# Samaretas/global-motion-estimation

Hardware: AMD Instinct MI355X
Metric: frame-pairs/s + achieved HBM GB/s, 720x480 bs=16 sw=16 exhaustive (higher is better)
Workload: dtype u8; 1 GPU; 720x480 synthetic luma, bs=16 sw=16 exhaustive MAE (BASELINE configs[1]); frame_distance=1, streams_per_gpu=1, collective=none, exchange=none in this run, multi_gpu_measured_by_builder=False

## Files before the change

global-motion-estimation_amd/csrc/bbme_sea.hip:

```cpp
#include "bbme_sea_common.h"

namespace {

using namespace sea;

constexpr int GUARD_NONE = 0, GUARD_ROWS = 1, GUARD_ALL = 2;
constexpr uint32_t PENALTY = 1u << 17;
constexpr uint32_t FIRST_INVALID_KEY = 65536u << 13;
template <int R, int GUARD>
__device__ __forceinline__ void lower_bounds(const uint64_t* sp0, int XQ, int prow, int q, uint32_t a01, uint32_t a23,
                                             int lo_r, int hi_r, int lo_c, int hi_c, uint32_t (&pkey)[R])
{
    constexpr bool SKIP = GUARD == GUARD_ALL && R >= 4;
#pragma unroll
    for (int k = 0; k < R; ++k) pkey[k] = 0xFFFFFFFFu;
    constexpr uint32_t penalty = PENALTY;
    uint32_t seed[R];
#pragma unroll
    for (int i = 0; i < R; ++i) {
        const int ri = prow * R + i;
        seed[i] = (GUARD == GUARD_NONE || SKIP || (ri >= lo_r && ri <= hi_r)) ? 0u : penalty;
    }
    const int nlo = lo_c - q * 4 * R, nhi = hi_c - q * 4 * R;
    const uint64_t* top = sp0;
    const uint64_t* bot = sp0 + 8 * XQ;
#pragma unroll
    for (int i = 0; i < R; ++i) {
        const int ri = prow * R + i;
        if (!SKIP || (ri >= lo_r && ri <= hi_r)) {
            uint64_t t[R + 2], b[R + 2];
#pragma unroll
            for (int k = 0; k < R + 2; ++k) { t[k] = top[k]; b[k] = bot[k]; }
#pragma unroll
            for (int k = 0; k < R; ++k) {
                if (SKIP && (4 * k > nhi || 4 * k + 3 < nlo)) continue;
#pragma unroll
                for (int e = 0; e < 4; ++e) {
                    if (SKIP && (4 * k + e < nlo || 4 * k + e > nhi)) continue;
                    const uint32_t sel = (e & 1) ? 0x07060302u : 0x05040100u;
                    const uint32_t tp = __builtin_amdgcn_perm((uint32_t)(t[k + 2] >> (32 * (e >> 1))), (uint32_t)(t[k] >> (32 * (e >> 1))), sel);
                    const uint32_t bt = __builtin_amdgcn_perm((uint32_t)(b[k + 2] >> (32 * (e >> 1))), (uint32_t)(b[k] >> (32 * (e >> 1))), sel);
                    const uint32_t start = (GUARD != GUARD_ALL || SKIP || 4 * k + e <= nhi) ? seed[i] : penalty;
                    const uint32_t lb = __builtin_amdgcn_sad_u16(tp, a01, __builtin_amdgcn_sad_u16(bt, a23, start));
                    pkey[k] = min(pkey[k], (lb << 13) + (uint32_t)((4 * k + e) * R + i));
                }
            }
        }
        top += XQ;
        bot += XQ;
    }
    if constexpr (GUARD != GUARD_NONE && !SKIP) {
#pragma unroll
        for (int k = 0; k < R; ++k)
            if (pkey[k] >= FIRST_INVALID_KEY || (GUARD == GUARD_ALL && 4 * k < nlo)) pkey[k] = 0xFFFFFFFFu;
    }
}

template <int R>
__device__ __forceinline__ uint32_t eval_patch_quad(const SeaGeo& d, int H, int W, const uint32_t* win, const uint32_t* anchor, uint32_t ent,
                                                    bool active, int sub, int trow, int bcol0, int NC)
{
    const int w2 = ent >> 25, l2 = (ent >> 19) & 63, k2 = (ent >> 16) & 7;
    const int wr2 = div_small(w2, d.magic_tc), wc2 = w2 - wr2 * d.tc;
    const int prow2 = l2 >> 2, q2 = l2 & 3;
    uint64_t acc[R];
#pragma unroll
    for (int i = 0; i < R; ++i) acc[i] = 0;
    if (active) {
        const uint32_t* lrow = win + (16 * wr2 + prow2 * R + 4 * sub) * d.pitch_dw + wc2 * 4 + q2 * R + k2;
        const uint32_t* an = anchor + w2 * ANCHOR_STRIDE + 16 * sub;
#pragma unroll
        for (int t = 0; t < R + 3; ++t) {
            uint64_t w[4];
#pragma unroll
            for (int s = 0; s < 4; ++s) w[s] = *(const u64_a4*)(lrow + t * d.pitch_dw + s);
#pragma unroll
            for (int i = 0; i < R; ++i) {
                const int a = t - i;
                if (a < 0 || a > 3) continue;
                const u32x4 ar = *(const u32x4*)(an + a * 4);
#pragma unroll
                for (int j = 0; j < 4; ++j)
                    acc[i] = __builtin_amdgcn_qsad_pk_u16_u8(w[j], ar[j], acc[i]);
            }
        }
    }
#pragma unroll
    for (int i = 0; i < R; ++i) {
        uint32_t lo = (uint32_t)acc[i], hi = (uint32_t)(acc[i] >> 32);
        lo += (uint32_t)__builtin_amdgcn_update_dpp(0, (int)lo, 0xB1, 0xF, 0xF, false);
        hi += (uint32_t)__builtin_amdgcn_update_dpp(0, (int)hi, 0xB1, 0xF, 0xF, false);
        lo += (uint32_t)__builtin_amdgcn_update_dpp(0, (int)lo, 0x4E, 0xF, 0xF, false);
        hi += (uint32_t)__builtin_amdgcn_update_dpp(0, (int)hi, 0x4E, 0xF, 0xF, false);
        asm volatile("" : "+v"(lo), "+v"(hi));
        acc[i] = ((uint64_t)hi << 32) | lo;
    }
    uint32_t key = 0xFFFFFFFFu;
    if (active) {
        const int c02 = (bcol0 + wc2) * 16, r02 = (trow * d.tr + wr2) * 16;
        const int lo_c = max(0, d.sw - c02), hi_c = min(NC - 1, W - 16 - c02 + d.sw);
        const int lo_r2 = max(0, d.sw - r02), hi_r2 = min(NC - 1, H - 16 - r02 + d.sw);
        const bool rows_inside2 = NC == 16 * R && lo_r2 == 0 && hi_r2 == NC - 1;
        const int ci = q2 * 4 * R + 4 * k2 + sub, ri0 = prow2 * R;
        const uint32_t shift = (uint32_t)(sub & 1) * 16u;
        if (rows_inside2 && lo_c == 0 && hi_c == NC - 1) {
#pragma unroll
            for (int i = 0; i < R; ++i) {
                const uint32_t word = (sub & 2) ? (uint32_t)(acc[i] >> 32) : (uint32_t)acc[i];
                const uint32_t sad = __builtin_amdgcn_ubfe(word, shift, 16u);
                key = min(key, (sad << 13) + (uint32_t)i);
            }
            key += (uint32_t)(ci * NC + ri0);
        } else if (ci >= lo_c && ci <= hi_c) {
#pragma unroll
            for (int i = 0; i < R; ++i) {
                const int ri = ri0 + i;
                if (ri < lo_r2 || ri > hi_r2) continue;
                const uint32_t word = (sub & 2) ? (uint32_t)(acc[i] >> 32) : (uint32_t)acc[i];
                const uint32_t sad = __builtin_amdgcn_ubfe(word, shift, 16u);
                key = min(key, (sad << 13) | (uint32_t)(ci * NC + ri));
            }
        }
        key = min(key, (uint32_t)__builtin_amdgcn_update_dpp(-1, (int)key, 0xB1, 0xF, 0xF, false));
        key = min(key, (uint32_t)__builtin_amdgcn_update_dpp(-1, (int)key, 0x4E, 0xF, 0xF, false));
    }
    return key;
}

template <int R, bool FIXED>
__device__ __forceinline__ bool tile_phases(const SeaGeo& d, uint32_t* lds, const Layout& L, int pair, int trow, int bcol0,
                                            uint32_t mine, uint32_t a01, uint32_t a23, int tid, int tile_id)
{
    constexpr bool E4 = R >= 3;
    const int T = blockDim.x;
    const int NC = 2 * d.sw + 16, XQ = d.xq;
    uint32_t* win = lds + L.win;
    uint32_t* anchor = lds + L.anchor;
    uint32_t* best = lds + L.best;
    uint32_t* count = lds + L.count;
    uint64_t* s8 = (uint64_t*)(lds + L.s8);
    uint32_t* work = lds + L.work;
    const int wave = __builtin_amdgcn_readfirstlane(tid >> 6);
    const int lane = tid & 63;
    const SeaArgs c = launch_args();
    const WaveBlock wb = wave_block(d, c, trow, bcol0, wave);
    const int brow = wb.brow, bcol = wb.bcol;
    const bool wave_ok = wb.ok;
    const int r0 = brow * 16, c0 = bcol * 16;
    const int prow = lane >> 2, q = lane & 3;

    box_sums8<R, FIXED>(d, win, s8, tid);
    __syncthreads();

    const int lo_r = max(0, d.sw - r0), hi_r = min(NC - 1, c->H - 16 - r0 + d.sw);
    const bool rows_inside = NC == 16 * R && lo_r == 0 && hi_r == NC - 1;
    uint32_t ub_key = 0xFFFFFFFFu;
    if (wave_ok) {
        const int lo_c = max(0, d.sw - c0), hi_c = min(NC - 1, c->W - 16 - c0 + d.sw);
        uint32_t pkey[R];
        const uint64_t* sp0 = s8 + (16 * wb.wr + prow * R) * XQ + wb.wc * 4 + q * R;
        const bool cols_inside = NC == 16 * R && lo_c == 0 && hi_c == NC - 1;
        if (rows_inside && cols_inside)
            lower_bounds<R, GUARD_NONE>(sp0, XQ, prow, q, a01, a23, lo_r, hi_r, lo_c, hi_c, pkey);
        else if (R <= 3 && cols_inside)
            lower_bounds<R, GUARD_ROWS>(sp0, XQ, prow, q, a01, a23, lo_r, hi_r, lo_c, hi_c, pkey);
        else
            lower_bounds<R, GUARD_ALL>(sp0, XQ, prow, q, a01, a23, lo_r, hi_r, lo_c, hi_c, pkey);
        const uint32_t first_idx = (uint32_t)((q * 4 * R) * NC + prow * R);
        uint32_t pkd[R], lb_key = 0xFFFFFFFFu;
#pragma unroll
        for (int k = 0; k < R; ++k) {
            pkd[k] = (pkey[k] & 0xFFFFE000u) | (first_idx + (uint32_t)(4 * k * NC));
            lb_key = min(lb_key, pkey[k]);
        }
        const uint32_t lane_lb = lb_key;
        if (lb_key != 0xFFFFFFFFu) lb_key += (uint32_t)lane << 7;
        lb_key = wave_min_u32(lb_key);
        {
            const int bl = (lb_key >> 7) & 63, loc = lb_key & 127;
            const int ce = loc / R, li = loc - ce * R;
            const int idx1 = ((bl & 3) * 4 * R + ce) * NC + (bl >> 2) * R + li;
            const int idx0 = d.sw * NC + d.sw;
            const int arow = lane >> 2, aj = lane & 3;
            uint32_t packed = 0;
#pragma unroll
            for (int which = 0; which < 2; ++which) {
                const int idx = which ? idx1 : idx0;
                const int ci = idx / NC, ri = idx - ci * NC;
                const int byte = wb.wc * 16 + ci + 4 * aj;
                const uint32_t* p = win + (16 * wb.wr + ri + arow) * d.pitch_dw + (byte >> 2);
                const uint32_t v = __builtin_amdgcn_alignbyte(p[1], p[0], (uint32_t)byte & 3u);
                packed += __builtin_amdgcn_sad_u8(v, mine, 0u) << (16 * which);
            }
            packed = wave_sum_u32(packed);
            ub_key = min(((packed & 0xFFFFu) << 13) | (uint32_t)idx0, ((packed >> 16) << 13) | (uint32_t)idx1);
            const int idxp = (int)(best[2 * wave + 1] & 0x1FFFu);
            const int cip = idxp / NC, rip = idxp - cip * NC;
            if (idxp != idx0 && idxp != idx1 && cip >= lo_c && cip <= hi_c && rip >= lo_r && rip <= hi_r) {
                const int byte = wb.wc * 16 + cip + 4 * aj;
                const uint32_t* p = win + (16 * wb.wr + rip + arow) * d.pitch_dw + (byte >> 2);
                const uint32_t v = __builtin_amdgcn_alignbyte(p[1], p[0], (uint32_t)byte & 3u);
                const uint32_t sadp = wave_sum_u32(__builtin_amdgcn_sad_u8(v, mine, 0u));
                ub_key = min(ub_key, (sadp << 13) | (uint32_t)idxp);
            }
        }
        uint32_t own_lim = 0;
        int n_w = 0;
        if constexpr (E4) {
            const int engage = c->engage;
            if (c->quota > 0 && __popcll(__ballot((lane_lb & 0xFFFFE000u) < ub_key)) > engage / 3) {
#pragma unroll
                for (int k = 0; k < R; ++k) n_w += __popcll(__ballot(pkd[k] < ub_key));
                if (n_w > engage) {
                    own_lim = first_round_limit(c, lb_key >> 13, ub_key >> 13, 13, [&](uint32_t lim) {
                        int c = 0;
#pragma unroll
                        for (int k = 0; k < R; ++k) c += __popcll(__ballot(pkd[k] < lim));
                        return c;
                    });
                    own_lim = min(own_lim, ub_key);
                    uint32_t* own = lds + L.own + 16 * wave;
                    int base_rank = 0;
                    uint32_t listed_here = 0;
#pragma unroll
                    for (int k = 0; k < R; ++k) {
                        const bool sel = pkd[k] < own_lim;
                        const unsigned long long m = __ballot(sel);
                        const int rank = base_rank + (int)__builtin_amdgcn_mbcnt_hi((uint32_t)(m >> 32), __builtin_amdgcn_mbcnt_lo((uint32_t)m, 0u));
                        if (sel && rank < 16) {
                            own[rank] = ((uint32_t)wave << 25) | ((uint32_t)lane << 19) | ((uint32_t)k << 16) | (pkd[k] >> 13);
                            listed_here |= 1u << k;
                        }
                        base_rank += __popcll(m);
                    }
                    const int n_own = min(base_rank, 16);
                    const bool act = (lane >> 2) < n_own;
                    const uint32_t ent = act ? own[lane >> 2] : 0u;
                    uint32_t key = eval_patch_quad<R>(d, c->H, c->W, win, anchor, ent, act, lane & 3, trow, bcol0, NC);
                    ub_key = min(ub_key, wave_min_u32(key));
#pragma unroll
                    for (int k = 0; k < R; ++k)
                        if (listed_here & (1u << k)) pkd[k] = 0xFFFFFFFFu;
                    if (lane == 0) atomicAdd(count + 5, (uint32_t)n_own);
                }
            }
        }
        if (lane == 0) best[2 * wave] = ub_key;
#pragma unroll
        for (int k = 0; k < R; ++k)
            if (pkd[k] < ub_key) {
                const uint32_t slot = atomicAdd(count, 1u);
                work[slot] = ((uint32_t)wave << 25) | ((uint32_t)lane << 19) | ((uint32_t)k << 16) | (pkd[k] >> 13);
            }
        if (own_lim) {
            int pushed = 0;
#pragma unroll
            for (int k = 0; k < R; ++k) pushed += __popcll(__ballot(pkd[k] < ub_key));
            if (lane == 0) atomicAdd(count + 4, (uint32_t)(n_w - pushed));
        }
    }
    __syncthreads();
    const SeaArgs ce = launch_args();
    if (ce->redo_list && (int)*count > ce->redo_threshold) {
        if (tid == 0) push_redo(ce, tile_id, (int)(blockIdx.x & 7));
        return true;
    }
    const int H = ce->H, W = ce->W;

    if constexpr (E4) {
        const int n = (int)*count;
        const int sub = lane & 3;
        for (int base = 0; base < n; base += T / 4) {
            const int e = base + (tid >> 2);
            bool active = e < n;
            uint32_t ent = 0;
            if (active) ent = work[e];
            const int w2 = ent >> 25, l2 = (ent >> 19) & 63, k2 = (ent >> 16) & 7;
            const int wr2 = div_small(w2, d.magic_tc), wc2 = w2 - wr2 * d.tc;
            const int prow2 = l2 >> 2, q2 = l2 & 3;
            active = active && (((ent & 0xFFFFu) << 13) | (uint32_t)((q2 * 4 * R + 4 * k2) * NC + prow2 * R)) < best[2 * w2];
            uint64_t acc[R];
    #pragma unroll
            for (int i = 0; i < R; ++i) acc[i] = 0;
            if (active) {
                const uint32_t* lrow = win + (16 * wr2 + prow2 * R + 4 * sub) * d.pitch_dw + wc2 * 4 + q2 * R + k2;
                const uint32_t* an = anchor + w2 * ANCHOR_STRIDE + 16 * sub;
    #pragma unroll
                for (int t = 0; t < R + 3; ++t) {
                    uint64_t w[4];
    #pragma unroll
                    for (int s = 0; s < 4; ++s) w[s] = *(const u64_a4*)(lrow + t * d.pitch_dw + s);
    #pragma unroll
                    for (int i = 0; i < R; ++i) {
                        const int a = t - i;
                        if (a < 0 || a > 3) continue;
                        const u32x4 ar = *(const u32x4*)(an + a * 4);
    #pragma unroll
                        for (int j = 0; j < 4; ++j)
                            acc[i] = __builtin_amdgcn_qsad_pk_u16_u8(w[j], ar[j], acc[i]);
                    }
                }
            }
    #pragma unroll
            for (int i = 0; i < R; ++i) {
                uint32_t lo = (uint32_t)acc[i], hi = (uint32_t)(acc[i] >> 32);
                lo += (uint32_t)__builtin_amdgcn_update_dpp(0, (int)lo, 0xB1, 0xF, 0xF, false);
                hi += (uint32_t)__builtin_amdgcn_update_dpp(0, (int)hi, 0xB1, 0xF, 0xF, false);
                lo += (uint32_t)__builtin_amdgcn_update_dpp(0, (int)lo, 0x4E, 0xF, 0xF, false);
                hi += (uint32_t)__builtin_amdgcn_update_dpp(0, (int)hi, 0x4E, 0xF, 0xF, false);
                asm volatile("" : "+v"(lo), "+v"(hi));
                acc[i] = ((uint64_t)hi << 32) | lo;
            }
            if (active) {
                const int c02 = (bcol0 + wc2) * 16, r02 = (trow * d.tr + wr2) * 16;
                const int lo_c = max(0, d.sw - c02), hi_c = min(NC - 1, W - 16 - c02 + d.sw);
                const int lo_r2 = max(0, d.sw - r02), hi_r2 = min(NC - 1, H - 16 - r02 + d.sw);
                const bool rows_inside2 = NC == 16 * R && lo_r2 == 0 && hi_r2 == NC - 1;
                const int ci = q2 * 4 * R + 4 * k2 + sub, ri0 = prow2 * R;
                const uint32_t shift = (uint32_t)(sub & 1) * 16u;
                uint32_t key = 0xFFFFFFFFu;
                if (rows_inside2 && lo_c == 0 && hi_c == NC - 1) {
    #pragma unroll
                    for (int i = 0; i < R; ++i) {
                        const uint32_t word = (sub & 2) ? (uint32_t)(acc[i] >> 32) : (uint32_t)acc[i];
                        const uint32_t sad = __builtin_amdgcn_ubfe(word, shift, 16u);
                        key = min(key, (sad << 13) + (uint32_t)i);
                    }
                    key += (uint32_t)(ci * NC + ri0);
                } else if (ci >= lo_c && ci <= hi_c) {
    #pragma unroll
                    for (int i = 0; i < R; ++i) {
                        const int ri = ri0 + i;
                        if (ri < lo_r2 || ri > hi_r2) continue;
                        const uint32_t word = (sub & 2) ? (uint32_t)(acc[i] >> 32) : (uint32_t)acc[i];
                        const uint32_t sad = __builtin_amdgcn_ubfe(word, shift, 16u);
                        key = min(key, (sad << 13) | (uint32_t)(ci * NC + ri));
                    }
                }
                key = min(key, (uint32_t)__builtin_amdgcn_update_dpp(-1, (int)key, 0xB1, 0xF, 0xF, false));
                key = min(key, (uint32_t)__builtin_amdgcn_update_dpp(-1, (int)key, 0x4E, 0xF, 0xF, false));
                if (sub == 0 && key != 0xFFFFFFFFu) atomicMin(&best[2 * w2], key);
            }
            __syncthreads();
        }
    } else {
        const int n = (int)*count;
        for (int base = 0; base < n; base += T) {
            const int e = base + tid;
            bool active = e < n;
            uint32_t ent = 0;
            if (active) {
                ent = work[e];
                const uint32_t first = (uint32_t)(((int)((ent >> 19) & 3) * 4 * R + 4 * (int)((ent >> 16) & 7)) * NC + (int)((ent >> 21) & 15) * R);
                active = (((ent & 0xFFFFu) << 13) | first) < best[2 * (ent >> 25)];
            }
            if (active) {
                const int w2 = ent >> 25, l2 = (ent >> 19) & 63, k2 = (ent >> 16) & 7;
                const int wr2 = div_small(w2, d.magic_tc), wc2 = w2 - wr2 * d.tc;
                const int prow2 = l2 >> 2, q2 = l2 & 3;
                const uint32_t* lrow = win + (16 * wr2 + prow2 * R) * d.pitch_dw + wc2 * 4 + q2 * R + k2;
                const uint32_t* an = anchor + w2 * ANCHOR_STRIDE;
                uint64_t acc[R];
    #pragma unroll
                for (int i = 0; i < R; ++i) acc[i] = 0;
    #pragma unroll
                for (int t = 0; t < R + 15; ++t) {
                    uint64_t w[4];
    #pragma unroll
                    for (int s = 0; s < 4; ++s) w[s] = *(const u64_a4*)(lrow + t * d.pitch_dw + s);
    #pragma unroll
                    for (int i = 0; i < R; ++i) {
                        const int a = t - i;
                        if (a < 0 || a > 15) continue;
                        const u32x4 ar = *(const u32x4*)(an + a * 4);
    #pragma unroll
                        for (int j = 0; j < 4; ++j)
                            acc[i] = __builtin_amdgcn_qsad_pk_u16_u8(w[j], ar[j], acc[i]);
                    }
                }
                const int c02 = (bcol0 + wc2) * 16, r02 = (trow * d.tr + wr2) * 16;
                const int lo_c = max(0, d.sw - c02), hi_c = min(NC - 1, W - 16 - c02 + d.sw);
                const int lo_r2 = max(0, d.sw - r02), hi_r2 = min(NC - 1, H - 16 - r02 + d.sw);
                const bool rows_inside2 = NC == 16 * R && lo_r2 == 0 && hi_r2 == NC - 1;
                const int ci0 = q2 * 4 * R + 4 * k2, ri0 = prow2 * R;
                uint32_t key = 0xFFFFFFFFu;
                if (rows_inside2 && lo_c == 0 && hi_c == NC - 1) {
    #pragma unroll
                    for (int e4 = 0; e4 < 4; ++e4)
    #pragma unroll
                        for (int i = 0; i < R; ++i) {
                            const uint32_t sad = (uint32_t)(acc[i] >> (16 * e4)) & 0xFFFFu;
                            key = min(key, (sad << 13) + (uint32_t)(e4 * NC + i));
                        }
                    key += (uint32_t)(ci0 * NC + ri0);
                } else {
    #pragma unroll
                    for (int e4 = 0; e4 < 4; ++e4) {
                        const int ci = ci0 + e4;
                        if (ci < lo_c || ci > hi_c) continue;
    #pragma unroll
                        for (int i = 0; i < R; ++i) {
                            const int ri = ri0 + i;
                            if (ri < lo_r2 || ri > hi_r2) continue;
                            const uint32_t sad = (uint32_t)(acc[i] >> (16 * e4)) & 0xFFFFu;
                            key = min(key, (sad << 13) | (uint32_t)(ci * NC + ri));
                        }
                    }
                }
                if (key != 0xFFFFFFFFu) atomicMin(&best[2 * w2], key);
            }
            __syncthreads();
        }

    }
    if (wave_ok && lane == 0) {
        const int idx = (int)(best[2 * wave] & 0x1FFF);
        const int ci = idx / NC, ri = idx - ci * NC;
        int32_t* o = ce->mf + (((long long)pair * ce->nbr + brow) * ce->nbc + bcol) * 2;
        o[0] = ci - d.sw;
        o[1] = ri - d.sw;
        best[2 * wave + 1] = (uint32_t)idx;
    }
    return false;
}

template <int R, bool FIXED = false>
struct MaeTile {
    struct Pre { uint32_t a01, a23; };
    static __device__ __forceinline__ Pre prep(uint32_t* lds, const Layout& L, int wave, int lane, bool wave_ok, uint32_t mine)
    {
        Pre p = { 0, 0 };
        if (wave_ok) {
            lds[L.anchor + wave * ANCHOR_STRIDE + lane] = mine;
            anchor_quadrants(mine, &p.a01, &p.a23);
        }
        return p;
    }
    static __device__ __forceinline__ bool phases(const SeaGeo& d, uint32_t* lds, const Layout& L, int pair, int trow, int bcol0,
                                                  uint32_t mine, const Pre& p, int tid, int tile_id)
    {
        return tile_phases<R, FIXED>(d, lds, L, pair, trow, bcol0, mine, p.a01, p.a23, tid, tile_id);
    }
    static __device__ __forceinline__ int probe_word(const Layout& L, int wave) { return L.best + 2 * wave + 1; }
};

template <int R>
__global__ void __launch_bounds__(1024) k_exh_sea16(SeaDev d)
{
    extern __shared__ uint32_t lds[];
    const SeaGeo g = d;
    one_tile<MaeTile<R>>(g, lds, layout_of(g, R));
}

template <int R, int NV, int GEO = 0>
__global__ void __launch_bounds__(1024, (R <= 3 ? 8 : 6)) k_exh_sea16p(SeaDev d)
{
    extern __shared__ uint32_t lds[];
    SeaGeo g = d;
    fix_geometry<R, GEO>(g);
    const Layout L = layout_of(g, R);
    if ((threadIdx.x & 63) == 0) lds[L.best + 2 * (threadIdx.x >> 6) + 1] = (uint32_t)(g.sw * (2 * g.sw + 16) + g.sw);
    persistent_tiles<NV, MaeTile<R, GEO != 0>>(g, lds, L);
}

struct MaeLaunch {
    static constexpr const char* persistent_name = "k_exh_sea16p";
    static constexpr const char* one_tile_name = "k_exh_sea16";
    static int no_plan()
    {
        gme_set_error("search window too large for LDS");
        return GME_ERR_ARG;
    }
    static void tables(SeaDev& d, const BbmeJob&) { d.sqbox = nullptr; d.sqbox_stride = 0; }
    static void ordered(SeaDev& d)
    {
        d.quota = getenv("GME_SEA_QUOTA") ? atoi(getenv("GME_SEA_QUOTA")) : SEA_DEFAULT_QUOTA;
        d.bisect = getenv("GME_SEA_BISECT") ? atoi(getenv("GME_SEA_BISECT")) : SEA_DEFAULT_BISECT;
        d.engage = getenv("GME_SEA_ENGAGE") ? atoi(getenv("GME_SEA_ENGAGE")) : SEA_DEFAULT_ENGAGE;
        if (d.engage < d.quota) d.engage = d.quota;
    }
    static bool fits(int R, int nv) { return R <= 1 || R >= 4 || nv <= 8; }
    template <int R, int NV, int GEO = 0>
    static void persistent(dim3 grid, dim3 block, size_t lds, hipStream_t s, const SeaDev& d)
    {
        hipLaunchKernelGGL((k_exh_sea16p<R, NV, GEO>), grid, block, lds, s, d);
    }
    template <int R>
    static void one_tile(dim3 grid, dim3 block, size_t lds, hipStream_t s, const SeaDev& d)
    {
        hipLaunchKernelGGL((k_exh_sea16<R>), grid, block, lds, s, d);
    }
};

}

bool bbme_sea_applies(int bs, int sw, int procedure, int pnorm)
{
    if (procedure != GME_SEARCH_EXHAUSTIVE || bs != 16 || pnorm != GME_NORM_MAE) return false;
    if (sw < 0 || sw % 4 != 0) return false;
    const int NC = 2 * sw + 16;
    return (NC + 15) / 16 <= 5 && NC * NC <= 8192 && !getenv("GME_FORCE_GENERIC") && !getenv("GME_EXH_BRUTE");
}

int launch_bbme_sea(gme_ctx* ctx, const BbmeJob& job, bool* handled)
{
    *handled = false;
    if (!bbme_sea_applies(job.bs, job.sw, job.procedure, job.pnorm)) return GME_OK;
    return launch_sea<MaeLaunch>(ctx, job, handled);
}
```

Baseline: 606,900 frame-pairs/s.

## Pair box sums vertically in SEA lower bounds and recover argmin candidate lazily

Reorders how the packed 16-bit box sums feed sad_u16 in the successive-elimination lower bound. Vertical pairing lets each perm'd top/bottom pair be reused across neighbouring candidate columns. The anchor quadrants are repacked to match. Per-candidate index keys are no longer built in the inner loop; the loop keeps only the minimum bound per lane, and a new ballot scan recovers the argmin candidate's position afterward. This cuts perm and key-packing ALU work in the hot loop, at the cost of an extra rescan for the minimum candidate. R=5 with NV=16 stays on horizontal pairing.

```diff
diff --git a/global-motion-estimation_amd/csrc/bbme_sea.hip b/global-motion-estimation_amd/csrc/bbme_sea.hip
--- a/global-motion-estimation_amd/csrc/bbme_sea.hip
+++ b/global-motion-estimation_amd/csrc/bbme_sea.hip
@@ -7,13 +7,24 @@
 constexpr int GUARD_NONE = 0, GUARD_ROWS = 1, GUARD_ALL = 2;
 constexpr uint32_t PENALTY = 1u << 17;
 constexpr uint32_t FIRST_INVALID_KEY = 65536u << 13;
-template <int R, int GUARD>
-__device__ __forceinline__ void lower_bounds(const uint64_t* sp0, int XQ, int prow, int q, uint32_t a01, uint32_t a23,
-                                             int lo_r, int hi_r, int lo_c, int hi_c, uint32_t (&pkey)[R])
+constexpr uint32_t FIRST_INVALID_BOUND = FIRST_INVALID_KEY >> 13;
+__device__ __forceinline__ uint32_t pair_u16(uint32_t t, uint32_t b, bool odd)
+{
+    return __builtin_amdgcn_perm(b, t, odd ? 0x07060302u : 0x05040100u);
+}
+template <bool VERT>
+__device__ __forceinline__ void candidate_pairs(uint32_t tl, uint32_t tr, uint32_t bl, uint32_t br, bool odd, uint32_t* first, uint32_t* second)
+{
+    *first = VERT ? pair_u16(tl, bl, odd) : pair_u16(tl, tr, odd);
+    *second = VERT ? pair_u16(tr, br, odd) : pair_u16(bl, br, odd);
+}
+template <int R, int GUARD, bool VERT>
+__device__ __forceinline__ void lower_bounds(const uint64_t* sp0, int XQ, int prow, int q, uint32_t pa, uint32_t pb,
+                                             int lo_r, int hi_r, int lo_c, int hi_c, uint32_t (&pmin)[R])
 {
     constexpr bool SKIP = GUARD == GUARD_ALL && R >= 4;
 #pragma unroll
-    for (int k = 0; k < R; ++k) pkey[k] = 0xFFFFFFFFu;
+    for (int k = 0; k < R; ++k) pmin[k] = 0xFFFFFFFFu;
     constexpr uint32_t penalty = PENALTY;
     uint32_t seed[R];
 #pragma unroll
@@ -31,18 +42,37 @@
             uint64_t t[R + 2], b[R + 2];
 #pragma unroll
             for (int k = 0; k < R + 2; ++k) { t[k] = top[k]; b[k] = bot[k]; }
-#pragma unroll
-            for (int k = 0; k < R; ++k) {
-                if (SKIP && (4 * k > nhi || 4 * k + 3 < nlo)) continue;
-#pragma unroll
-                for (int e = 0; e < 4; ++e) {
-                    if (SKIP && (4 * k + e < nlo || 4 * k + e > nhi)) continue;
-                    const uint32_t sel = (e & 1) ? 0x07060302u : 0x05040100u;
-                    const uint32_t tp = __builtin_amdgcn_perm((uint32_t)(t[k + 2] >> (32 * (e >> 1))), (uint32_t)(t[k] >> (32 * (e >> 1))), sel);
-                    const uint32_t bt = __builtin_amdgcn_perm((uint32_t)(b[k + 2] >> (32 * (e >> 1))), (uint32_t)(b[k] >> (32 * (e >> 1))), sel);
-                    const uint32_t start = (GUARD != GUARD_ALL || SKIP || 4 * k + e <= nhi) ? seed[i] : penalty;
-                    const uint32_t lb = __builtin_amdgcn_sad_u16(tp, a01, __builtin_amdgcn_sad_u16(bt, a23, start));
-                    pkey[k] = min(pkey[k], (lb << 13) + (uint32_t)((4 * k + e) * R + i));
+            if constexpr (SKIP || !VERT) {
+#pragma unroll
+                for (int k = 0; k < R; ++k) {
+                    if (SKIP && (4 * k > nhi || 4 * k + 3 < nlo)) continue;
+#pragma unroll
+                    for (int e = 0; e < 4; ++e) {
+                        if (SKIP && (4 * k + e < nlo || 4 * k + e > nhi)) continue;
+                        const int sh = 32 * (e >> 1);
+                        uint32_t first, second;
+                        candidate_pairs<VERT>((uint32_t)(t[k] >> sh), (uint32_t)(t[k + 2] >> sh), (uint32_t)(b[k] >> sh), (uint32_t)(b[k + 2] >> sh), e & 1, &first, &second);
+                        const uint32_t start = (GUARD != GUARD_ALL || SKIP || 4 * k + e <= nhi) ? seed[i] : penalty;
+                        pmin[k] = min(pmin[k], __builtin_amdgcn_sad_u16(first, pa, __builtin_amdgcn_sad_u16(second, pb, start)));
+                    }
+                }
+            } else {
+                uint32_t vp[R + 2][4];
+#pragma unroll
+                for (int k = 0; k < R; ++k) {
+#pragma unroll
+                    for (int m = (k < 2 ? k : k + 2); m <= k + 2; m += 2)
+#pragma unroll
+                        for (int e = 0; e < 4; ++e)
+                            vp[m][e] = pair_u16((uint32_t)(t[m] >> (32 * (e >> 1))), (uint32_t)(b[m] >> (32 * (e >> 1))), e & 1);
+                    uint32_t lb[4];
+#pragma unroll
+                    for (int e = 0; e < 4; ++e) {
+                        const uint32_t start = (GUARD != GUARD_ALL || 4 * k + e <= nhi) ? seed[i] : penalty;
+                        lb[e] = __builtin_amdgcn_sad_u16(vp[k][e], pa, __builtin_amdgcn_sad_u16(vp[k + 2][e], pb, start));
+                    }
+                    pmin[k] = min(min(pmin[k], lb[0]), lb[1]);
+                    pmin[k] = min(min(pmin[k], lb[2]), lb[3]);
                 }
             }
         }
@@ -52,8 +82,39 @@
     if constexpr (GUARD != GUARD_NONE && !SKIP) {
 #pragma unroll
         for (int k = 0; k < R; ++k)
-            if (pkey[k] >= FIRST_INVALID_KEY || (GUARD == GUARD_ALL && 4 * k < nlo)) pkey[k] = 0xFFFFFFFFu;
-    }
+            if (pmin[k] >= FIRST_INVALID_BOUND || (GUARD == GUARD_ALL && 4 * k < nlo)) pmin[k] = 0xFFFFFFFFu;
+    }
+}
+
+template <int R, bool VERT>
+__device__ __forceinline__ int min_bound_candidate(const uint64_t* s8blk, int XQ, int NC, int bl, uint32_t mb, uint32_t pa, uint32_t pb,
+                                                   int lo_r, int hi_r, int lo_c, int hi_c, int lane)
+{
+    const int col0 = (bl & 3) * 4 * R, row0 = (bl >> 2) * R;
+    const uint16_t* tab = (const uint16_t*)(s8blk + row0 * XQ + (bl & 3) * R);
+    int loc = 0;
+    bool found = false;
+#pragma unroll
+    for (int base = 0; base < 4 * R * R; base += 64) {
+        const int l = base + lane;
+        const int ce = l / R, li = l - ce * R;
+        bool hit = false;
+        if (4 * R * R - base >= 64 || l < 4 * R * R) {
+            const uint16_t* p = tab + li * 4 * XQ + ce;
+            uint32_t first, second;
+            candidate_pairs<VERT>(p[0], p[8], p[32 * XQ], p[32 * XQ + 8], false, &first, &second);
+            const uint32_t lb = __builtin_amdgcn_sad_u16(first, pa, __builtin_amdgcn_sad_u16(second, pb, 0u));
+            const int ci = col0 + ce, ri = row0 + li;
+            hit = lb == mb && ci >= lo_c && ci <= hi_c && ri >= lo_r && ri <= hi_r;
+        }
+        const unsigned long long m = __ballot(hit);
+        if (!found && m) {
+            loc = base + __builtin_ctzll(m);
+            found = true;
+        }
+    }
+    const int ce = loc / R, li = loc - ce * R;
+    return (col0 + ce) * NC + row0 + li;
 }
 
 template <int R>
@@ -127,9 +188,9 @@
     return key;
 }
 
-template <int R, bool FIXED>
+template <int R, bool FIXED, bool VERT>
 __device__ __forceinline__ bool tile_phases(const SeaGeo& d, uint32_t* lds, const Layout& L, int pair, int trow, int bcol0,
-                                            uint32_t mine, uint32_t a01, uint32_t a23, int tid, int tile_id)
+                                            uint32_t mine, uint32_t pa, uint32_t pb, int tid, int tile_id)
 {
     constexpr bool E4 = R >= 3;
     const int T = blockDim.x;
@@ -157,29 +218,29 @@
     uint32_t ub_key = 0xFFFFFFFFu;
     if (wave_ok) {
         const int lo_c = max(0, d.sw - c0), hi_c = min(NC - 1, c->W - 16 - c0 + d.sw);
-        uint32_t pkey[R];
-        const uint64_t* sp0 = s8 + (16 * wb.wr + prow * R) * XQ + wb.wc * 4 + q * R;
+        uint32_t pmin[R];
+        const uint64_t* s8blk = s8 + 16 * wb.wr * XQ + wb.wc * 4;
+        const uint64_t* sp0 = s8blk + prow * R * XQ + q * R;
         const bool cols_inside = NC == 16 * R && lo_c == 0 && hi_c == NC - 1;
         if (rows_inside && cols_inside)
-            lower_bounds<R, GUARD_NONE>(sp0, XQ, prow, q, a01, a23, lo_r, hi_r, lo_c, hi_c, pkey);
+            lower_bounds<R, GUARD_NONE, VERT>(sp0, XQ, prow, q, pa, pb, lo_r, hi_r, lo_c, hi_c, pmin);
         else if (R <= 3 && cols_inside)
-            lower_bounds<R, GUARD_ROWS>(sp0, XQ, prow, q, a01, a23, lo_r, hi_r, lo_c, hi_c, pkey);
+            lower_bounds<R, GUARD_ROWS, VERT>(sp0, XQ, prow, q, pa, pb, lo_r, hi_r, lo_c, hi_c, pmin);
         else
-            lower_bounds<R, GUARD_ALL>(sp0, XQ, prow, q, a01, a23, lo_r, hi_r, lo_c, hi_c, pkey);
+            lower_bounds<R, GUARD_ALL, VERT>(sp0, XQ, prow, q, pa, pb, lo_r, hi_r, lo_c, hi_c, pmin);
         const uint32_t first_idx = (uint32_t)((q * 4 * R) * NC + prow * R);
-        uint32_t pkd[R], lb_key = 0xFFFFFFFFu;
+        uint32_t pkd[R], lane_min = 0xFFFFFFFFu;
 #pragma unroll
         for (int k = 0; k < R; ++k) {
-            pkd[k] = (pkey[k] & 0xFFFFE000u) | (first_idx + (uint32_t)(4 * k * NC));
-            lb_key = min(lb_key, pkey[k]);
-        }
-        const uint32_t lane_lb = lb_key;
-        if (lb_key != 0xFFFFFFFFu) lb_key += (uint32_t)lane << 7;
+            pkd[k] = (pmin[k] << 13) | (first_idx + (uint32_t)(4 * k * NC));
+            lane_min = min(lane_min, pmin[k]);
+        }
+        const uint32_t lane_lb = lane_min << 13;
+        uint32_t lb_key = lane_min != 0xFFFFFFFFu ? lane_lb + ((uint32_t)lane << 7) : 0xFFFFFFFFu;
         lb_key = wave_min_u32(lb_key);
         {
-            const int bl = (lb_key >> 7) & 63, loc = lb_key & 127;
-            const int ce = loc / R, li = loc - ce * R;
-            const int idx1 = ((bl & 3) * 4 * R + ce) * NC + (bl >> 2) * R + li;
+            const int idx1 = min_bound_candidate<R, VERT>(s8blk, XQ, NC, (int)(lb_key >> 7) & 63, lb_key >> 13, pa, pb,
+                                                          lo_r, hi_r, lo_c, hi_c, lane);
             const int idx0 = d.sw * NC + d.sw;
             const int arow = lane >> 2, aj = lane & 3;
             uint32_t packed = 0;
@@ -208,7 +269,7 @@
         int n_w = 0;
         if constexpr (E4) {
             const int engage = c->engage;
-            if (c->quota > 0 && __popcll(__ballot((lane_lb & 0xFFFFE000u) < ub_key)) > engage / 3) {
+            if (c->quota > 0 && __popcll(__ballot(lane_lb < ub_key)) > engage / 3) {
 #pragma unroll
                 for (int k = 0; k < R; ++k) n_w += __popcll(__ballot(pkd[k] < ub_key));
                 if (n_w > engage) {
@@ -424,22 +485,25 @@
     return false;
 }
 
-template <int R, bool FIXED = false>
+template <int R, bool FIXED = false, bool VERT = true>
 struct MaeTile {
-    struct Pre { uint32_t a01, a23; };
+    struct Pre { uint32_t pa, pb; };
     static __device__ __forceinline__ Pre prep(uint32_t* lds, const Layout& L, int wave, int lane, bool wave_ok, uint32_t mine)
     {
         Pre p = { 0, 0 };
         if (wave_ok) {
             lds[L.anchor + wave * ANCHOR_STRIDE + lane] = mine;
-            anchor_quadrants(mine, &p.a01, &p.a23);
+            uint32_t a01, a23;
+            anchor_quadrants(mine, &a01, &a23);
+            p.pa = VERT ? pair_u16(a01, a23, false) : a01;
+            p.pb = VERT ? pair_u16(a01, a23, true) : a23;
         }
         return p;
     }
     static __device__ __forceinline__ bool phases(const SeaGeo& d, uint32_t* lds, const Layout& L, int pair, int trow, int bcol0,
                                                   uint32_t mine, const Pre& p, int tid, int tile_id)
     {
-        return tile_phases<R, FIXED>(d, lds, L, pair, trow, bcol0, mine, p.a01, p.a23, tid, tile_id);
+        return tile_phases<R, FIXED, VERT>(d, lds, L, pair, trow, bcol0, mine, p.pa, p.pb, tid, tile_id);
     }
     static __device__ __forceinline__ int probe_word(const Layout& L, int wave) { return L.best + 2 * wave + 1; }
 };
@@ -451,6 +515,8 @@
     const SeaGeo g = d;
     one_tile<MaeTile<R>>(g, lds, layout_of(g, R));
 }
+
+constexpr bool vertical_pairs(int R, int NV) { return !(R == 5 && NV == 16); }
 
 template <int R, int NV, int GEO = 0>
 __global__ void __launch_bounds__(1024, (R <= 3 ? 8 : 6)) k_exh_sea16p(SeaDev d)
@@ -460,7 +526,7 @@
     fix_geometry<R, GEO>(g);
     const Layout L = layout_of(g, R);
     if ((threadIdx.x & 63) == 0) lds[L.best + 2 * (threadIdx.x >> 6) + 1] = (uint32_t)(g.sw * (2 * g.sw + 16) + g.sw);
-    persistent_tiles<NV, MaeTile<R, GEO != 0>>(g, lds, L);
+    persistent_tiles<NV, MaeTile<R, GEO != 0, vertical_pairs(R, NV)>>(g, lds, L);
 }
 
 struct MaeLaunch {
```

Result: faster. 620,300 frame-pairs/s, median of 6 (+2.2%).
